# michaelwillett/GPU-ICP-SLAM

Hardware: AMD Instinct MI355X
Metric: particle-scan evals/sec (1081 beams x N particles), full particleFilter step, KD path (higher is better)
Workload: dtype f32; 1 GPU; synthetic 1081-beam scans, 100000 particles/GPU, 100000-point KD map, full SLAM step (disperse+score+weights+ICP/SVD+map update+resample); particles_global=100000, parallelism=particles sharded x1, map replicated, kd_size_end=193011

## Files before the change

gpu-icp-slam_amd/binding.py:

```python
import ctypes as C
import os

import numpy as np

from . import build as _build

NODE_DTYPE = np.dtype(
    [("axis", "<i4"), ("left", "<i4"), ("right", "<i4"), ("parent", "<i4"),
     ("x", "<f4"), ("y", "<f4"), ("z", "<f4"), ("w", "<f4")])
PARTICLE_DTYPE = np.dtype(
    {"names": ["x", "y", "theta", "w", "cluster", "map"],
     "formats": ["<f4", "<f4", "<f4", "<f4", "u1", "<u8"],
     "offsets": [0, 4, 8, 12, 16, 24], "itemsize": 32})

SYMBOLS = [
    "pfslam_default_config", "pfslam_create", "pfslam_destroy", "pfslam_last_error", "pfslam_device_count",
    "pfslam_set_stream", "pfslam_synchronize", "pfslam_step", "pfslam_step_grid", "pfslam_shard_disperse", "pfslam_shard_score", "pfslam_shard_weights", "pfslam_shard_finish", "pfslam_shard_stream", "pfslam_get_pose", "pfslam_get_particles",
    "pfslam_get_map", "pfslam_get_grid", "pfslam_get_trace", "pfslam_get_cells", "pfslam_set_map",
    "pfslam_set_particles", "pfslam_shift_particles", "pfslam_set_scan", "pfslam_set_pose", "pfslam_set_grid", "pfslam_motion_update",
    "pfslam_score_kd", "pfslam_measurement_update", "pfslam_icp", "pfslam_update_map_kd", "pfslam_resample",
    "pfslam_score_grid", "pfslam_update_map_grid", "pfslam_traverse", "pfslam_measurement_local",
    "pfslam_measurement_apply", "pfslam_device_ptr", "pfslam_time_score_kd", "pfslam_set_variant", "pfslam_set_lag",
    "pfslam_kd_create", "pfslam_kd_insert_list", "pfslam_kd_insert_node", "pfslam_kd_balance", "pfslam_set_timing", "pfslam_get_timers", "pfslam_resample_plan", "pfslam_resample_gather", "pfslam_maybe_balance", "pfslam_kd_size", "pfslam_topology_update", "pfslam_find_walls",
    "pfslam_check_loop_closure", "pfslam_get_topology", "pfslam_set_topology", "pfslam_get_closures", "pfslam_score_census", "pfslam_set_census", "pfslam_get_census_log", "pfslam_ubench_gather", "pfslam_plan_stats", "pfslam_cell_stats", "pfslam_kd_parallel_sort", "pfslam_kd_sort_threads", "pfslam_kd_whole_node",
# ... 565 lines not shown

    def traverse(self, xyz):
        xyz = np.ascontiguousarray(xyz, dtype=np.float32).reshape(-1, 3)
        best = np.empty(len(xyz), np.int32)
        _chk(self.L.pfslam_traverse(self._h, _p(xyz), len(xyz), _p(best)), "pfslam_traverse")
        return best

    def debug_math(self, which, x):
        x = np.ascontiguousarray(x, dtype=np.float32).ravel()
        out = np.empty(len(x) * (2 if which in (0, 6, 7) else 1), np.float32)
        _chk(self.L.pfslam_debug_math(self._h, which, _p(x), len(x), _p(out)), "pfslam_debug_math")
        if which == 6:
            return out.view(np.int32).reshape(-1, 2)
        return out.reshape(-1, 2) if which in (0, 7) else out

    @property
    def pose(self):
        out = np.zeros(3, np.float32)
        _chk(self.L.pfslam_get_pose(self._h, _p(out)), "pfslam_get_pose")
        return out

    def particles(self):
        ptr, n = C.c_void_p(), C.c_int()
        _chk(self.L.pfslam_get_particles(self._h, C.byref(ptr), C.byref(n)), "pfslam_get_particles")
        buf = (C.c_char * (32 * n.value)).from_address(ptr.value)
        return np.frombuffer(buf, dtype=PARTICLE_DTYPE).copy()

    def map(self):
        ptr, n = C.c_void_p(), C.c_int()
        _chk(self.L.pfslam_get_map(self._h, C.byref(ptr), C.byref(n)), "pfslam_get_map")
# ... 29 lines not shown
```

gpu-icp-slam_amd/build.py:

```python
import fcntl
import hashlib
import os
import shutil
import subprocess

HERE = os.path.dirname(os.path.abspath(__file__))
CSRC = os.path.join(HERE, "csrc")
OBJ = os.path.join(HERE, "build")
LIB = os.path.join(HERE, "libpfslam_hip.so")
INC = os.path.join("..", "..", "include", "pfslam.h")
UNITS = {
    "pfslam_hip.hip": ["pf_math.h", "kd_device.h", "kd_cells.hip.inc", "pfslam_stages.hip.inc", "pfslam_frame.hip.inc", INC],
    "kd_host.cpp": [INC],
}
FLAGS = ["--offload-arch=gfx950", "-O3", "-std=c++17", "-ffp-contract=off", "-fPIC",
         "-Wall", "-Wno-unused-function", "-Wno-unused-result"] + os.environ.get("PFSLAM_EXTRA_FLAGS", "").split()


def hipcc():
    for c in (os.environ.get("HIPCC"), "/opt/rocm/bin/hipcc", shutil.which("hipcc")):
        if c and os.path.exists(c):
            return c
    raise RuntimeError("hipcc not found: libpfslam_hip.so cannot be built (there is no CPU fallback)")


def _digest(files):
    h = hashlib.sha1(" ".join(FLAGS).encode())
# ... 58 lines not shown
```

gpu-icp-slam_amd/csrc/kd_device.h:

```cpp
#pragma once
#include "pf_math.h"


namespace pf {

struct KdView {
    const uint4 *hot;
    const float *z;
    const int *parent;
    const float *w;
    int planar;
};

struct KdCensus {
    unsigned long long trips;
    unsigned long long lanes;
    unsigned long long tests;
    unsigned long long test_lanes;
    unsigned long long uniform;
    unsigned long long prefix;
    unsigned long long redesc;
    unsigned long long redesc_noop;
};

// ... 30 lines not shown
}
__device__ __forceinline__ int kd_load_i32(kd_rsrc_t r, int idx)
{
    return (int)__builtin_amdgcn_raw_buffer_load_b32(r, idx << 2, 0, 0);
}
__device__ __forceinline__ int kd_load_i32_bytes(kd_rsrc_t r, int byte_offset)
{
    return (int)__builtin_amdgcn_raw_buffer_load_b32(r, byte_offset, 0, 0);
}
__device__ __forceinline__ uint4 kd_load_hot_at(kd_rsrc_t r, int base, int imm)
{
    typedef unsigned u32x4 __attribute__((ext_vector_type(4)));
    const u32x4 v = __builtin_amdgcn_raw_buffer_load_b128(r, base + imm, 0, 0);
    return make_uint4(v.x, v.y, v.z, v.w);
}
#else
struct kd_rsrc_t { const void *base; };
__device__ kd_rsrc_t kd_rsrc(const void *base);
__device__ uint4 kd_load_hot(kd_rsrc_t r, int idx);
__device__ int kd_load_i32(kd_rsrc_t r, int idx);
__device__ int kd_load_i32_bytes(kd_rsrc_t r, int byte_offset);
__device__ uint4 kd_load_hot_at(kd_rsrc_t r, int base, int imm);
#endif

struct KdCensusLocal { unsigned trips, lanes, tests, test_lanes, uniform, prefix, redesc, redesc_noop; };
__device__ __forceinline__ void census_add(unsigned &ev, unsigned &lanes)
{
    const unsigned long long ex = __builtin_amdgcn_read_exec();
    if ((int)(threadIdx.x & 63) == __ffsll((long long)ex) - 1) ev++;
    lanes++;
}
__device__ __forceinline__ void census_flush(const KdCensusLocal &c, KdCensus *out)
{
// ... 110 lines not shown
        if (BOUNDED && head >= bound) head = -1;
        if (CENSUS) {
            in_redesc = true;
            census->redesc++;
        }
    }
    return bestIdx;
}

template <bool PLANAR, bool CENSUS = false>
__device__ __forceinline__ int kd_nearest_ref(const KdView &t, float px, float py, float pz, KdCensusLocal *census = nullptr)
{
    return kd_resume<PLANAR, CENSUS>(t, px, py, pz, INFINITY, 0, 0, census);
}

#define PF_PLAN_CAND 7
struct KdPlanRow {
    int n_cand;
    int resume;
    int path_len;
    float range;
    float4 cand[PF_PLAN_CAND];
};
static_assert(sizeof(KdPlanRow) == 16 + 16 * PF_PLAN_CAND, "plan row layout");

struct KdGroupBox { float xlo, xhi, ylo, yhi, tlo, thi; int count, pad; };

__device__ __forceinline__ float lidar_angle(int n)
{
    const float PI_F = 3.1415926535897932384626422832795028841971f;
// ... 23 lines not shown
```

gpu-icp-slam_amd/csrc/pfslam_frame.hip.inc:

```

#define PF_FRAME_RING 4
enum { PF_FS_BOUND = 0, PF_FS_WALKED = 4, PF_FS_TICKET = 8, PF_FS_ICP = 9, PF_FS_WORDS = 16 };
enum { PF_WC_WALLS = 0, PF_WC_NEW, PF_WC_FLAGS, PF_WC_SIZE, PF_WC_WORDS = 4 };

enum { PF_FL_REDUCED = 0, PF_FL_TREE, PF_FL_ORDER, PF_FL_ICP, PF_FL_SCAN, PF_FL_FTAIL, PF_FL_POSEG , PF_FL_WORDS = 8 };
__device__ __forceinline__ void flag_store(int *word, int ticket) { __hip_atomic_store(word, ticket, __ATOMIC_RELEASE, __HIP_MEMORY_SCOPE_AGENT); }
__device__ __forceinline__ bool flag_wait(const int *word, int ticket, int *err)
{
    const unsigned long long t0 = wall_clock64(), limit = g_gate_ticks;
    while (__hip_atomic_load(word, __ATOMIC_ACQUIRE, __HIP_MEMORY_SCOPE_AGENT) - ticket < 0) {
        __builtin_amdgcn_s_sleep(8);
        if (wall_clock64() - t0 > limit) {
            if (err) __hip_atomic_store(err, ticket, __ATOMIC_RELAXED, __HIP_MEMORY_SCOPE_SYSTEM);
            return false;
        }
    }
    return true;
}
__global__ void k_gate(const int *__restrict__ word, int ticket, int *__restrict__ err)
{
    if (threadIdx.x == 0) flag_wait(word, ticket, err);
}
__global__ void k_gate_signal(int *__restrict__ done_word, int done_ticket, const int *__restrict__ word, int ticket, int *__restrict__ err)
{
// ... 431 lines not shown
#pragma unroll
        for (int q = k >> 1; q > 0; q >>= 1) {
            const uint32_t other = (uint32_t)__shfl_xor((int)key, q, 64);
            const bool asc = (lane & k) == 0, lower = (lane & q) == 0;
            key = (lower == asc) ? min(key, other) : max(key, other);
        }
    runs_g[j] = key;
    keys_s[j] = 0xFFFFFFFFu;
    if (probe && blockIdx.x == 0 && lane == 0) probe[PB_WALLS_KEYS - PB_WALLS] = wall_clock64();
}

template <bool PLANAR>
__global__ __launch_bounds__(64) void k_walls_rank_traverse(const uint32_t *__restrict__ runs_g, int sort_n, const float *__restrict__ pose, int dimx, float resx,
                                                            float resy, float scalex, float scaley, pf::KdView tree, uint32_t *__restrict__ keys_s,
                                                            float2 *__restrict__ xy_s, int *__restrict__ c2_s, int *__restrict__ leaf_s,
                                                            int *__restrict__ new_s, unsigned long long *__restrict__ probe, int split)
{
    pf_stamp(probe);
    extern __shared__ uint32_t s_dyn[];
    uint32_t *runs = s_dyn;
    const int lane = threadIdx.x, n_runs = sort_n >> 6, mine = blockIdx.x / split, per = 64 / split, pos = (blockIdx.x % split) * per + lane;
    for (int i = lane; i < sort_n; i += 64) runs[i] = runs_g[i];
    __syncthreads();
    if (lane >= per) return;
    const int i = mine * 64 + pos;
    const uint32_t key = runs[i];
    if (key == 0xFFFFFFFFu) return;
    int rank = pos;
    bool dup = pos > 0 && runs[i - 1] == key;
    for (int r0 = 0; r0 < n_runs; r0 += 4) {
        int lo[4] = {0, 0, 0, 0};
// ... 9 lines not shown
        for (int step = 32; step >= 1; step >>= 1)
#pragma unroll
            for (int u = 0; u < 4; u++)
                if (on[u]) lo[u] += (runs[(r0 + u) * 64 + lo[u] + step - 1] <= pk[u]) ? step : 0;
#pragma unroll
        for (int u = 0; u < 4; u++)
            if (on[u]) {
                const int cnt = lo[u] + ((lo[u] == 63 && runs[(r0 + u) * 64 + 63] <= pk[u]) ? 1 : 0);
                rank += cnt;
                if (r0 + u < mine && cnt > 0 && runs[(r0 + u) * 64 + cnt - 1] == key) dup = true;
            }
    }
    if (dup) return;
    const float4 p = cell_to_point((int)key, dimx, resx, resy, scalex, scaley, pose[0], pose[1]);
    int leaf;
    const int b = pf::kd_resume<PLANAR, false, true>(tree, p.x, p.y, p.z, INFINITY, 0, 0, nullptr, &leaf);
    const float cellDiag = pf::fsqrt(resx * resx + resy * resy), minDist = cellDiag / 2.0f;
    keys_s[rank] = key;
    xy_s[rank] = make_float2(p.x, p.y);
    c2_s[rank] = b;
    leaf_s[rank] = leaf;
    new_s[rank] = node_dist(tree, b, p) > minDist ? 1 : 0;
}

template <bool PLANAR>
__global__ __launch_bounds__(256) void k_free_traverse(float4 *__restrict__ free_pts, int *__restrict__ free_idx, int free_cap, int wall_cap,
                                                       const int *__restrict__ counts, pf::KdView tree, int zero_tail, float *kw, float resx,
                                                       float resy, const int *__restrict__ bound_ptr, unsigned long long *__restrict__ probe)
{
    pf_stamp(probe);
    const int n_wall = min(counts[0], wall_cap), n_free = min(counts[1], free_cap);
// ... 7 lines not shown
        }
        const int b = pf::kd_resume<PLANAR, false, false, true>(tree, p.x, p.y, p.z, INFINITY, 0, 0, nullptr, nullptr, bound);
        free_idx[i] = b;
        const bool hit = node_dist(tree, b, p) < cellDiag;
        if (zero_tail && i >= n_wall) {
            const unsigned long long m = __ballot(hit);
            if (hit && (int)(threadIdx.x & 63) == __ffsll((long long)m) - 1) map_weight_add(kw, b, PF_FREE_WEIGHT, __popcll(m));
        } else if (hit) map_weight_add(kw, b, PF_FREE_WEIGHT);
    }
}

__global__ __launch_bounds__(1024) void k_wall_weights(const float4 *__restrict__ wall_pts, const int *__restrict__ wall_cell, int wall_cap,
                                                      const int *__restrict__ wall_c2, const int *__restrict__ counts,
                                                      const int *__restrict__ wcounts, pf::KdView tree, float *kw, float resx, float resy,
                                                      const float *__restrict__ pose, HostHeader *__restrict__ hdr, int seq,
                                                      unsigned long long *__restrict__ probe)
{
    pf_stamp(probe);
    const int n_wall = min(counts[0], wall_cap);
    const float cellDiag = pf::fsqrt(resx * resx + resy * resy);
    for (int i = threadIdx.x; i < n_wall; i += 1024) {
        const int b = wall_c2[i];
        if (node_dist(tree, b, wall_pts[i]) < cellDiag) map_weight_add(kw, b, PF_OCCUPIED_WEIGHT);
    }
    if (threadIdx.x != 0 || !hdr) return;
    const int bad = counts[0] != wcounts[PF_WC_WALLS] ? PF_HDR_INTERNAL : 0;
    hdr->n_wall = counts[0];
    hdr->n_free = counts[1];
    hdr->n_new = wcounts[PF_WC_NEW];
    hdr->kd_size = wcounts[PF_WC_SIZE];
    hdr->flags = wcounts[PF_WC_FLAGS] | bad;
    for (int k = 0; k < 4; k++) hdr->pose[k] = pose[k];
    __threadfence_system();
// ... 710 lines not shown
        const int cx = (int)roundf(0.5f * h->dimx + h->cfg.map_res_x / 2), cy = (int)roundf(0.5f * h->dimy + h->cfg.map_res_y / 2);
        const int wait_poseg = c.multi ? 1 : 0;
#define PF_WALLS_ARGS dim3(1), dim3(1024), lds, C, (const float *)h->scan, (const pf::BeamParts *)h->beam_angle, h->nb, sort_n, c.psrc, h->start, h->pose, c.stats_next, \
                      cx, cy, h->dimx, h->dimy, h->cfg.map_res_x, h->cfg.map_res_y, h->cfg.map_scale_x, h->cfg.map_scale_y, c.tv, h->hot, h->parent, h->kz, h->kw,   \
                      h->kd_state, h->kd_cap, sort_n, h->wall_c2, h->wcounts, h->fs + PF_FS_BOUND + ((seq + 1) & 3), (const int *)h->cell_state, h->cell_touched
        if (h->planar == 0) {
            hipLaunchKernelGGL(k_walls<0>, PF_WALLS_ARGS, PB(PB_WALLS), h->wall_xy2, h->wall_leaf2, h->wall_new2, gates ? fl : (int *)nullptr, seq, h->gate_err_dev,
                               (const uint32_t *)nullptr, (const int *)nullptr, wait_poseg, h->trig);
        } else {
            hipLaunchKernelGGL(k_wall_runs, dim3(sort_n / 64), dim3(64), 0, C, (const float *)h->scan, (const pf::BeamParts *)h->beam_angle, h->nb, c.psrc, h->start, h->pose,
                               c.stats_next, cx, cy, h->dimx, h->dimy, h->cfg.map_res_x, h->cfg.map_res_y, h->wall_runs, h->wall_keys_s, PB(PB_WALLS),
                               gates ? fl : (int *)nullptr, seq, h->gate_err_dev, wait_poseg, h->trig);
            const int walls_split = 4;
            hipLaunchKernelGGL(k_walls_rank_traverse<true>, dim3(sort_n / 64 * walls_split), dim3(64), (size_t)sort_n * 4, C, (const uint32_t *)h->wall_runs, sort_n,
                               (const float *)h->pose, h->dimx, h->cfg.map_res_x, h->cfg.map_res_y, h->cfg.map_scale_x, h->cfg.map_scale_y, c.tv, h->wall_keys_s,
                               h->wall_xy2, h->wall_c2s, h->wall_leaf2, h->wall_new2, PB(PB_WALLS_REP), walls_split);
            hipLaunchKernelGGL(k_walls<3>, PF_WALLS_ARGS, PB(PB_WALLS), h->wall_xy2, h->wall_leaf2, h->wall_new2, (int *)nullptr, seq, (int *)nullptr,
                               (const uint32_t *)h->wall_keys_s, (const int *)h->wall_c2s);
        }
#undef PF_WALLS_ARGS
        HIPCHK(hipGetLastError());
        if (!gates) HIPCHK(hipEventRecord(h->ev_tree2, C));
        const int recut = h->cells_passes > 0 && h->cells_passes % PF_CELLS_RECUT_EVERY == 0 ? 1 : 0;
        if (recut) HIPCHK(hipMemsetAsync(h->cell_state + PF_CS_POOL, 0, 4, C));
        hipLaunchKernelGGL(k_cells_update<true>, dim3(PF_CELLS_GRID), dim3(64), 0, C, c.tv, c.geo, h->cell_tab, (const int *)h->cell_list, h->cell_state, h->cell_pool,
                           h->cell_rec, h->cells_gen, (const int *)h->cell_touched, (int)(h->cells_passes & 15), recut, 0,
                           CellPass{nullptr, nullptr, h->fs + PF_FS_WALKED + ((seq - (sync_cells ? 0 : lag)) & 3), nullptr, h->fault}, PB(PB_UPDATE),
                           gates ? fl + PF_FL_TREE : (int *)nullptr, seq);
        HIPCHK(hipGetLastError());
        h->cells_passes++;
    }
// ... 70 lines not shown
        hipLaunchKernelGGL(k_count_cells, dim3(nblk), dim3(256), 0, F, h->free_mask, h->wall_mask, M, h->blk_cnt);
        hipLaunchKernelGGL(k_scatter_cells, dim3(nblk), dim3(256), 0, F, h->free_mask, h->wall_mask, M, h->blk_cnt, h->counts, h->dimx, h->cfg.map_res_x,
                           h->cfg.map_res_y, h->cfg.map_scale_x, h->cfg.map_scale_y, h->pose, h->wall_cell, h->wall_pts, h->max_wall, h->free_cell,
                           h->free_pts, h->max_free, 1, c.psrc);
        h->masks_cleared = true;
        if (h->planar)
            hipLaunchKernelGGL(k_free_traverse<true>, dim3(1024), dim3(256), 0, F, h->free_pts, h->free_c, h->max_free, h->max_wall, (const int *)h->counts, c.tv,
                               h->cfg.free_upload_bug, h->kw, h->cfg.map_res_x, h->cfg.map_res_y, (const int *)(h->fs + PF_FS_BOUND + s4), PB(PB_FREE));
        else
            hipLaunchKernelGGL(k_free_traverse<false>, dim3(1024), dim3(256), 0, F, h->free_pts, h->free_c, h->max_free, h->max_wall, (const int *)h->counts, c.tv,
                               h->cfg.free_upload_bug, h->kw, h->cfg.map_res_x, h->cfg.map_res_y, (const int *)(h->fs + PF_FS_BOUND + s4), PB(PB_FREE));
        HIPCHK(hipGetLastError());
        FV_EDGE_WAIT(F, PF_FL_TREE, h->ev_tree2, 0);
        hipLaunchKernelGGL(k_wall_weights, dim3(1), dim3(1024), 0, F, (const float4 *)h->wall_pts, (const int *)h->wall_cell, h->max_wall, (const int *)h->wall_c2,
                           (const int *)h->counts, (const int *)h->wcounts, c.tv, h->kw, h->cfg.map_res_x, h->cfg.map_res_y, (const float *)h->pose, c.hdr, seq,
                           PB(PB_WALLW));
        HIPCHK(hipGetLastError());
        h->ftail_recorded = !c.ftail_gate;
        if (!c.ftail_gate) HIPCHK(hipEventRecord(h->ev_ftail, F));
    }
    h->pipe_live = true;
    h->plan_valid = false;
    h->cells_valid = true;
    h->mirror_stale = true;
    h->stats_clean = false;
    h->icp_delta_ready = false;
    h->scan_front_done = false;
    pfslam_handle::Frame fr{seq, frame, 0, true, true};
    fr.gtheta = c.multi;
    h->in_flight.push_back(fr);
    while ((int)h->in_flight.size() > (h->topo_in_step == 1 ? 0 : h->lag)) CHK(consume_frame(h));
// ... 14 lines not shown
```

gpu-icp-slam_amd/csrc/pfslam_hip.hip:

```cpp
#include "../../include/pfslam.h"
#include "kd_device.h"
#include "pf_math.h"

#include <hip/hip_runtime.h>

#include <algorithm>
#include <atomic>
#include <deque>
#include <thread>
#include <cmath>
#include <cstdio>
#include <chrono>
#include <cstring>
#include <string>
#include <vector>

#define PF_LIDAR_RANGE 20.0f
#define PF_RANGE_NEVER 28.4f
#define PF_FREE_WEIGHT (-1)
#define PF_OCCUPIED_WEIGHT 4
#define PF_EFFECTIVE_PARTICLES .7
#define PF_CLAMP_VAL 113.0f
#define PF_SVD_EPSILON 0.00001f
#define PF_SUM_TILE 4096
// ... 51 lines not shown
    bool own_stream = false;
    int variant = 0;
    float *pblk = nullptr, *pblk2 = nullptr;
    float *x = nullptr, *y = nullptr, *th = nullptr, *w = nullptr, *wm = nullptr;
    float *x2 = nullptr, *y2 = nullptr, *th2 = nullptr;
    float *gw = nullptr, *gpose = nullptr;
    bool own_global = false;
    long long *gkeys = nullptr, *mkeys = nullptr;
    float *gtheta = nullptr;
    float *scan = nullptr;
    float *scan_base = nullptr;
    int kd_size = 0, kd_cap = 0, planar = 1;
    uint4 *hot = nullptr;
    int *parent = nullptr;
    float *kz = nullptr, *kw = nullptr;
    std::vector<pfslam_node> h_nodes;
    bool integral_w = true;
    float w_absmax = 113.0f;
    float *fit = nullptr, *partial = nullptr;
    size_t partial_elems = 0;
    unsigned *mkey = nullptr;
    int *order2 = nullptr;
    int *cells = nullptr;
    int64_t *stats = nullptr;
    float *pose = nullptr;
    float *start = nullptr;
    float h_pose[3] = {0, 0, 0};
    float *icp_tar = nullptr, *icp_cor = nullptr, *icp_dbg = nullptr;
    uint8_t *free_mask = nullptr, *wall_mask = nullptr;
    int *blk_cnt = nullptr;
// ... 522 lines not shown
    if (i < n) {
        const unsigned c = cell[i];
        order[tile_off[c >> 10] + atomicAdd(&cursor[c], 1)] = i;
    }
}

template <bool PLANAR>
__global__ __launch_bounds__(256) void k_traverse(const float *__restrict__ xyz, int n, pf::KdView tree,
                                                  int *__restrict__ best)
{
    int i = blockIdx.x * 256 + threadIdx.x;
    if (i >= n) return;
    best[i] = pf::kd_nearest_ref<PLANAR>(tree, xyz[3 * i], xyz[3 * i + 1], xyz[3 * i + 2]);
}

__global__ void k_debug_math(int which, const float *__restrict__ in, int n, float *__restrict__ out)
{
    int i = blockIdx.x * blockDim.x + threadIdx.x;
    if (i >= n) return;
    if (which == 0) {
        float s, c;
        pf::sincosf_spec(in[i], s, c);
        out[2 * i] = s;
        out[2 * i + 1] = c;
    } else if (which == 1) {
        out[i] = pf::erfcinvf_spec(in[i]);
    } else if (which == 2) {
        out[i] = pf::asinf_spec(in[i]);
    } else if (which == 3) {
        out[i] = pf::rsqrtf_spec(in[i]);
// ... 119 lines not shown
        CHK(dalloc(&h->gw, (size_t)h->world * S)); CHK(dalloc(&h->gpose, (size_t)h->world * 3 * S));
        h->own_global = true;
        const unsigned long long ticks = PF_GATE_TICKS_SHARDED;
        HIPCHK(hipMemcpyToSymbol(HIP_SYMBOL(g_gate_ticks), &ticks, sizeof(ticks)));
    } else {
        h->gw = h->w;
        h->gpose = h->pblk;
    }
    CHK(dalloc(&h->scan_base, (size_t)h->nb * PF_HDR_SLOTS));
    CHK(dalloc(&h->beam_angle, (size_t)h->nb));
    hipLaunchKernelGGL(k_beam_angles, dim3((h->nb + 255) / 256), dim3(256), 0, h->stream, h->beam_angle, h->nb);
    HIPCHK(hipGetLastError());
    h->scan = h->scan_base;
    CHK(dalloc(&h->hot, (size_t)h->kd_cap)); CHK(dalloc(&h->parent, (size_t)h->kd_cap));
    CHK(dalloc(&h->kz, (size_t)h->kd_cap)); CHK(dalloc(&h->kw, (size_t)h->kd_cap));
    CHK(dalloc(&h->fit, n)); CHK(dalloc(&h->fit_i, n));
    CHK(dalloc(&h->mkey, n)); CHK(dalloc(&h->order2, n));
    CHK(dalloc(&h->cells, (size_t)2 * PF_CELLS_MAX + PF_CELLS_MAX / 1024));
    HIPCHK(hipMemsetAsync(h->cells, 0, ((size_t)2 * PF_CELLS_MAX + PF_CELLS_MAX / 1024) * sizeof(int), h->stream));
    CHK(dalloc(&h->stats, 8)); CHK(dalloc(&h->pose, 4)); CHK(dalloc(&h->start, 4));
    CHK(dalloc(&h->icp_tar, (size_t)h->nb * 4)); CHK(dalloc(&h->icp_cor, (size_t)h->nb * 4)); CHK(dalloc(&h->icp_dbg, 64));
    CHK(dalloc(&h->free_mask, 2 * M));
    h->wall_mask = h->free_mask + M;
    h->max_wall = h->nb;
    h->max_free = (int)std::min<size_t>(M, (size_t)h->nb * (size_t)std::max(h->dimx, h->dimy));
    CHK(dalloc(&h->blk_cnt, 2 * ((M + 4095) / 4096) + 8));
    CHK(dalloc(&h->wall_cell, (size_t)h->max_wall)); CHK(dalloc(&h->free_cell, (size_t)h->max_free));
    CHK(dalloc(&h->wall_pts, (size_t)h->max_wall)); CHK(dalloc(&h->free_pts, (size_t)h->max_free));
    CHK(dalloc(&h->wall_c, (size_t)h->max_wall)); CHK(dalloc(&h->free_c, (size_t)h->max_free));
    CHK(dalloc(&h->counts, 8));
// ... 65 lines not shown
        const std::string msg = g_err;
        pfslam_destroy(h);
        g_err = msg;
        return rc;
    }
    *out = h;
    return 0;
}

extern "C" int pfslam_destroy(pfslam_handle *h)
{
    if (!h) return 0;
    (void)hipSetDevice(h->cfg.device);
    (void)settle(h);
    if (h->stream) (void)hipStreamSynchronize(h->stream);
    void *bufs[] = {h->pblk, h->pblk2, h->w, h->wm, h->gkeys, h->mkeys, h->gtheta, h->scan_base, h->hot, h->parent, h->kz, h->kw,
                    h->fit, h->fit_i, h->partial, h->mkey, h->order2, h->cells, h->stats, h->pose, h->start, h->icp_tar, h->icp_cor, h->icp_dbg,
                    h->free_mask, h->blk_cnt, h->wall_cell, h->free_cell, h->wall_pts, h->free_pts,
                    h->wall_c, h->free_c, h->counts, h->tile_r, h->tile_r2, h->sums, h->cdf,
                    h->chunk_max, h->tile_tot, h->tile_off, h->tile_pmax, h->src, h->est_part, h->grid, h->d_count, h->wall_leaf, h->kd_state, h->d_sigma};
    for (void *b : bufs)
        if (b) (void)hipFree(b);
    if (h->own_global) {
        (void)hipFree(h->gw); (void)hipFree(h->gpose);
    }
    if (h->pin_tree) (void)hipHostFree(h->pin_tree);
    if (h->h_hdr) (void)hipHostFree(h->h_hdr);
    if (h->h_scan) (void)hipHostFree(h->h_scan);
    if (h->ev0) (void)hipEventDestroy(h->ev0);
    if (h->ev1) (void)hipEventDestroy(h->ev1);
    if (h->aux) { (void)hipStreamSynchronize(h->aux); (void)hipStreamDestroy(h->aux); }
// ... 140 lines not shown
    const int per = (n + nt - 1) / nt;
    for (int t = 0; t < nt; t++) th.emplace_back([=] { fn(std::min(n, t * per), std::min(n, (t + 1) * per), t); });
    for (auto &t : th) t.join();
}

static int upload_tree(pfslam_handle *h, const pfslam_node *nodes, int n, std::vector<pfslam_node> *own = nullptr)
{
    if (n > h->kd_cap) return fail("map larger than kd_capacity");
    if (n == 0) {
        h->h_nodes.clear();
        h->kd_size = 0;
        h->mirror_n = 0;
        h->mirror_stale = false;
        h->cells_wipe_pending = true;
        HIPCHK(hipMemsetAsync(h->kd_state, 0, 16, h->stream));
        HIPCHK(hipStreamSynchronize(h->stream));
        return 0;
    }
    std::vector<uint4> hot_v;
    std::vector<int> par_v;
    std::vector<float> z_v, w_v;
    if (!h->pin_tree) {
        void *p = nullptr;
        if (hipHostMalloc(&p, (size_t)h->kd_cap * 28, hipHostMallocDefault) == hipSuccess) h->pin_tree = p;
        else (void)hipGetLastError();
    }
    uint4 *hot;
    int *par;
    float *z, *w;
    if (h->pin_tree) {
// ... 52 lines not shown
            if (planar && nd.axis == 2) memcpy(&z[i], &nd.left, 4);
        }
    });
    HIPCHK(hipMemcpyAsync(h->hot, hot, (size_t)n * 16, hipMemcpyHostToDevice, h->stream));
    HIPCHK(hipMemcpyAsync(h->parent, par, (size_t)n * 4, hipMemcpyHostToDevice, h->stream));
    HIPCHK(hipMemcpyAsync(h->kz, z, (size_t)n * 4, hipMemcpyHostToDevice, h->stream));
    HIPCHK(hipMemcpyAsync(h->kw, w, (size_t)n * 4, hipMemcpyHostToDevice, h->stream));
    float wabs;
    {
        const int wb = wmax_bits.load();
        memcpy(&wabs, &wb, 4);
        wabs = std::max(wabs, PF_CLAMP_VAL);
    }
    const int state[4] = {n, planar, integral ? (int)std::min(wabs, 1e9f) : 0, lattice ? 1 : 0};
    HIPCHK(hipMemcpyAsync(h->kd_state, state, 16, hipMemcpyHostToDevice, h->stream));
    if (own && own->data() == nodes && (int)own->size() == n) h->h_nodes.swap(*own);
    else h->h_nodes.assign(nodes, nodes + n);
    HIPCHK(hipStreamSynchronize(h->stream));
    h->kd_size = n;
    h->mirror_n = n;
    h->mirror_stale = false;
    h->planar = planar;
    h->integral_w = integral;
    h->w_absmax = wabs;
    h->lattice_ok = lattice;
    h->cells_wipe_pending = true;
    h->pipe_live = false;
    h->cells_suspended = false;
    h->cells_full_frame = -1;
    return 0;
// ... 923 lines not shown
    CHK(settle(h));
    const int per = which == 0 || which == 6 || which == 7 ? 2 : 1;
    float *d_in = nullptr, *d_out = nullptr;
    CHK(dalloc(&d_in, (size_t)n));
    CHK(dalloc(&d_out, (size_t)n * per));
    HIPCHK(hipMemcpyAsync(d_in, in_host, (size_t)n * 4, hipMemcpyHostToDevice, h->stream));
    hipLaunchKernelGGL(k_debug_math, dim3((n + 255) / 256), dim3(256), 0, h->stream, which, d_in, n, d_out);
    HIPCHK(hipGetLastError());
    HIPCHK(hipMemcpyAsync(out_host, d_out, (size_t)n * per * 4, hipMemcpyDeviceToHost, h->stream));
    HIPCHK(hipStreamSynchronize(h->stream));
    HIPCHK(hipFree(d_in));
    HIPCHK(hipFree(d_out));
    return 0;
}

extern "C" int pfslam_device_ptr(pfslam_handle *h, int which, void **ptr, size_t *bytes)
{
    if (!h || !ptr || !bytes) return fail("pfslam_device_ptr: bad argument");
    const size_t n = h->n;
    switch (which) {
    case 0: *ptr = h->stats; *bytes = 64; break;
    case 1: *ptr = h->fit; *bytes = n * 4; break;
    case 2: *ptr = h->x; *bytes = n * 4; break;
    case 3: *ptr = h->y; *bytes = n * 4; break;
    case 4: *ptr = h->th; *bytes = n * 4; break;
    case 5: *ptr = h->w; *bytes = (size_t)h->stride * 4; break;
    case 6: *ptr = h->tile_r; *bytes = ((n + PF_SUM_TILE - 1) / PF_SUM_TILE) * 4; break;
    case 7: *ptr = h->scan; *bytes = (size_t)h->nb * 4; break;
    case 8: *ptr = h->start; *bytes = 16; break;
    case 9: *ptr = h->pose; *bytes = 16; break;
// ... 26 lines not shown
```

gpu-icp-slam_amd/csrc/pfslam_stages.hip.inc:

```

__device__ __forceinline__ long long wave_max_i64(long long v)
{
    for (int off = 32; off >= 1; off >>= 1) {
        long long o = __shfl_xor(v, off, 64);
        v = o > v ? o : v;
    }
    return v;
}
__device__ __forceinline__ float wave_max_f32(float v)
{
    for (int off = 32; off >= 1; off >>= 1) v = fmaxf(v, __shfl_xor(v, off, 64));
    return v;
}
template <typename F>
__device__ __forceinline__ float wave_sum_canonical(int n, F elem)
{
    const int lane = threadIdx.x & 63;
    float acc = 0.0f;
    for (int i = lane; i < n; i += 64) acc = acc + elem(i);
    for (int off = 32; off >= 1; off >>= 1) acc = acc + __shfl_xor(acc, off, 64);
    return acc;
}

__device__ __forceinline__ int f32_to_ordered(float f)
// ... 2548 lines not shown
    return rc;
}
extern "C" int pfslam_shard_balance_adopt(pfslam_handle *h)
{
    if (!h) return fail("null handle");
    HIPCHK(hipSetDevice(h->cfg.device));
    CHK(settle(h));
    int st[4] = {0, 0, 0, 0};
    HIPCHK(hipMemcpyAsync(st, h->kd_state, 16, hipMemcpyDeviceToHost, h->stream));
    HIPCHK(hipStreamSynchronize(h->stream));
    if (st[0] != h->kd_size) return fail("pfslam_shard_balance_adopt: the broadcast map has " + std::to_string(st[0]) + " nodes, this rank's " + std::to_string(h->kd_size));
    h->planar = st[1];
    h->integral_w = st[2] != 0;
    h->w_absmax = st[2] != 0 ? (float)st[2] : 113.0f;
    h->lattice_ok = st[3] != 0;
    h->mirror_n = 0;
    h->mirror_stale = true;
    h->cells_wipe_pending = true;
    return 0;
}

extern "C" int pfslam_maybe_balance(pfslam_handle *h, int frame)
{
    if (!h) return fail("null handle");
    HIPCHK(hipSetDevice(h->cfg.device));
    CHK(settle(h));
    return balance_if_due(h, frame);
}
extern "C" int pfslam_kd_size(pfslam_handle *h)
{
// ... 231 lines not shown
```

gpu-icp-slam_amd/csrc/pfslam_testhooks.h:

```cpp
#ifndef PFSLAM_TESTHOOKS_H
#define PFSLAM_TESTHOOKS_H
#include "../../include/pfslam.h"
#ifdef __cplusplus
extern "C" {
#endif
int pfslam_debug_math(pfslam_handle *h, int which, const float *in_host, int n, float *out_host);
#ifdef __cplusplus
}
#endif
#endif
```

Before: 173.5 million particle-scan evals/s.

## Prefetch grandchild nodes via hint table in wall-rank KD traversal

Adds a per-node hint table holding grandchild indices. The table is rebuilt when the map is set or adopted and patched incrementally after inserts in the wall-weights kernel. The wall-rank traversal kernel now uses a paired walk that loads the next node and both candidate grandchildren in parallel, which shortens the chain of dependent loads in the KD descent. In exchange it issues more memory traffic per step, adds hint maintenance work, and depends on the hints staying current after tree updates.

```diff
diff --git a/gpu-icp-slam_amd/binding.py b/gpu-icp-slam_amd/binding.py
--- a/gpu-icp-slam_amd/binding.py
+++ b/gpu-icp-slam_amd/binding.py
@@ -603,6 +603,21 @@
             return out.view(np.int32).reshape(-1, 2)
         return out.reshape(-1, 2) if which in (0, 7) else out
 
+    def debug_walk_paired(self, xyz, hint_mode=0):
+        xyz = np.ascontiguousarray(xyz, dtype=np.float32).reshape(-1, 3)
+        out = [np.empty(len(xyz), np.int32) for _ in range(4)]
+        f = self.L.pfslam_debug_walk_paired
+        f.argtypes = [C.c_void_p, C.c_void_p, C.c_int, C.c_int] + [C.c_void_p] * 4
+        _chk(f(self._h, _p(xyz), len(xyz), hint_mode, *[_p(o) for o in out]), "pfslam_debug_walk_paired")
+        return tuple(out)
+
+    def debug_hints(self):
+        out = np.zeros(3, np.int64)
+        f = self.L.pfslam_debug_hints
+        f.argtypes = [C.c_void_p, C.c_void_p]
+        _chk(f(self._h, _p(out)), "pfslam_debug_hints")
+        return int(out[0]), int(out[1]), int(out[2])
+
     @property
     def pose(self):
         out = np.zeros(3, np.float32)
diff --git a/gpu-icp-slam_amd/build.py b/gpu-icp-slam_amd/build.py
--- a/gpu-icp-slam_amd/build.py
+++ b/gpu-icp-slam_amd/build.py
@@ -10,7 +10,7 @@
 LIB = os.path.join(HERE, "libpfslam_hip.so")
 INC = os.path.join("..", "..", "include", "pfslam.h")
 UNITS = {
-    "pfslam_hip.hip": ["pf_math.h", "kd_device.h", "kd_cells.hip.inc", "pfslam_stages.hip.inc", "pfslam_frame.hip.inc", INC],
+    "pfslam_hip.hip": ["pf_math.h", "kd_device.h", "kd_hint.h", "kd_cells.hip.inc", "pfslam_stages.hip.inc", "pfslam_frame.hip.inc", INC],
     "kd_host.cpp": [INC],
 }
 FLAGS = ["--offload-arch=gfx950", "-O3", "-std=c++17", "-ffp-contract=off", "-fPIC",
diff --git a/gpu-icp-slam_amd/csrc/kd_device.h b/gpu-icp-slam_amd/csrc/kd_device.h
--- a/gpu-icp-slam_amd/csrc/kd_device.h
+++ b/gpu-icp-slam_amd/csrc/kd_device.h
@@ -1,5 +1,6 @@
 #pragma once
 #include "pf_math.h"
+#include "kd_hint.h"
 
 
 namespace pf {
@@ -68,9 +69,21 @@
     const u32x4 v = __builtin_amdgcn_raw_buffer_load_b128(r, base + imm, 0, 0);
     return make_uint4(v.x, v.y, v.z, v.w);
 }
+__device__ __forceinline__ kd_rsrc_t kd_rsrc_n(const void *base, unsigned bytes)
+{
+    return __builtin_amdgcn_make_buffer_rsrc(const_cast<void *>(base),  0, (int)bytes, 0x00020000);
+}
+__device__ __forceinline__ int4 kd_load_hint(kd_rsrc_t r, int idx)
+{
+    typedef unsigned u32x4 __attribute__((ext_vector_type(4)));
+    const u32x4 v = __builtin_amdgcn_raw_buffer_load_b128(r, idx << 4, 0, 0);
+    return make_int4((int)v.x, (int)v.y, (int)v.z, (int)v.w);
+}
 #else
 struct kd_rsrc_t { const void *base; };
 __device__ kd_rsrc_t kd_rsrc(const void *base);
+__device__ kd_rsrc_t kd_rsrc_n(const void *base, unsigned bytes);
+__device__ int4 kd_load_hint(kd_rsrc_t r, int idx);
 __device__ uint4 kd_load_hot(kd_rsrc_t r, int idx);
 __device__ int kd_load_i32(kd_rsrc_t r, int idx);
 __device__ int kd_load_i32_bytes(kd_rsrc_t r, int byte_offset);
@@ -211,6 +224,128 @@
     return kd_resume<PLANAR, CENSUS>(t, px, py, pz, INFINITY, 0, 0, census);
 }
 
+struct KdStep { uint4 rec; int zw; int4 hint; int idx; };
+
+template <bool PLANAR>
+__device__ __forceinline__ int kd_walk_paired(const KdView &t, const int4 *hint, int cap, float px, float py, float pz, int *leaf_slot)
+{
+    const kd_rsrc_t hot_rsrc = kd_rsrc_n(t.hot, (unsigned)cap * 16u), z_rsrc = kd_rsrc_n(t.z, (unsigned)cap * 4u),
+                    hint_rsrc = kd_rsrc_n(hint, (unsigned)cap * 16u);
+    auto fetch = [&](int i) {
+        KdStep s;
+        s.rec = kd_load_hot(hot_rsrc, i);
+        s.zw = kd_load_i32(z_rsrc, i);
+        s.hint = kd_load_hint(hint_rsrc, i);
+        s.idx = i;
+        return s;
+    };
+    float sBest = INFINITY;
+    int bestIdx = 0, prevBest = -1, leaf = -1;
+    bool leaf_open = true;
+    bool went_left = false;
+    KdStep prev = {make_uint4(0u, 0u, 0u, 0u), 0, make_int4(-1, -1, -1, -1), -1};
+    KdStep par = prev;
+    auto visit = [&](const KdStep &n) -> int {
+        const uint4 nd = n.rec;
+        const int head = n.idx;
+        typedef float f32x2 __attribute__((ext_vector_type(2)));
+        const f32x2 nxy = {__uint_as_float(nd.x), __uint_as_float(nd.y)};
+        const f32x2 pxy = {px, py};
+        const f32x2 d = nxy - pxy;
+        const f32x2 dd = d * d;
+        float s = dd.x + dd.y;
+        float dz = 0.0f;
+        int zleft = 0;
+        if (!PLANAR) {
+            const float zraw = __int_as_float(n.zw);
+            const float nz = t.planar ? 0.0f : zraw;
+            zleft = n.zw;
+            dz = nz - pz;
+            s = s + dz * dz;
+        }
+        const float sGuard = sBest * PF_GUARD_K;
+        bool take = s < sGuard;
+        const bool inBand = (s < sBest) != take;
+        if (__builtin_amdgcn_ballot_w64(inBand) != 0ull) {
+            float sb = sBest;
+            asm volatile("" : "+v"(sb));
+            take = take | (inBand && fsqrt(s) < fsqrt(sb));
+        }
+        sBest = take ? s : sBest;
+        bestIdx = take ? head : bestIdx;
+        if (take) par = prev;
+        const uint32_t axis = nd.z >> 30;
+        float da = axis == 0 ? d.x : d.y;
+        if (!PLANAR) da = axis == 2 ? dz : da;
+        const bool lt = da > 0.0f;
+        int left = hot_left(nd.z);
+        if (!PLANAR) left = (t.planar && axis == 2) ? zleft : left;
+        if (leaf_open) leaf = head * 2 + ((lt && !(PLANAR && axis == 2)) ? 0 : 1);
+        prev = n;
+        went_left = lt;
+        return lt ? left : (int)nd.w;
+    };
+    const KdStep root = fetch(0);
+    int c = visit(root);
+    int pL = went_left ? root.hint.x : root.hint.z, pR = went_left ? root.hint.y : root.hint.w;
+    for (;;) {
+        while (c >= 0) {
+            const KdStep a = fetch(c), l = fetch(pL < 0 ? 0 : pL), r = fetch(pR < 0 ? 0 : pR);
+            const int g = visit(a);
+            if (g < 0) break;
+            KdStep b;
+            if (g == pL) b = l;
+            else if (g == pR) b = r;
+            else b = fetch(g);
+            c = visit(b);
+            pL = went_left ? b.hint.x : b.hint.z;
+            pR = went_left ? b.hint.y : b.hint.w;
+        }
+        if (leaf_open) {
+            leaf_open = false;
+            *leaf_slot = leaf;
+        }
+        if (bestIdx == prevBest) break;
+        prevBest = bestIdx;
+        const float bestDist = fsqrt(sBest);
+        if (par.idx < 0) break;
+        const uint4 nd = par.rec;
+        const float nx = __uint_as_float(nd.x), ny = __uint_as_float(nd.y);
+        const uint32_t axis = nd.z >> 30;
+        float pa = axis == 0 ? px : py, na = axis == 0 ? nx : ny;
+        float hd;
+        bool lt;
+        int left = hot_left(nd.z);
+        bool true_left = false;
+        if (PLANAR) {
+            hd = axis < 2 ? fabsf(pa - na) : 0.0f;
+            lt = (pa < na) & (axis < 2);
+            if (axis == 2) {
+                left = par.zw;
+                true_left = true;
+            }
+        } else {
+            if (axis == 2) {
+                const float zraw = __int_as_float(par.zw);
+                pa = pz;
+                na = t.planar ? 0.0f : zraw;
+                if (t.planar) {
+                    left = par.zw;
+                    true_left = true;
+                }
+            }
+            hd = fabsf(pa - na);
+            lt = pa < na;
+        }
+        if (!(hd < bestDist)) break;
+        c = lt ? (int)nd.w : left;
+        pL = lt ? par.hint.z : true_left ? -1 : par.hint.x;
+        pR = lt ? par.hint.w : true_left ? -1 : par.hint.y;
+        prev = par;
+    }
+    return bestIdx;
+}
+
 #define PF_PLAN_CAND 7
 struct KdPlanRow {
     int n_cand;
diff --git a/gpu-icp-slam_amd/csrc/kd_hint.h b/gpu-icp-slam_amd/csrc/kd_hint.h
--- /dev/null
+++ b/gpu-icp-slam_amd/csrc/kd_hint.h
@@ -0,0 +1,28 @@
+#pragma once
+#include <stdint.h>
+
+#if defined(__HIPCC__)
+#define KD_HINT_HD __host__ __device__ __forceinline__
+#else
+#define KD_HINT_HD inline
+#endif
+
+struct KdHint { int ll, lr, rl, rr; };
+
+KD_HINT_HD int kd_hint_left(uint32_t la) { return ((int)(la << 2)) >> 2; }
+
+template <class Hot>
+KD_HINT_HD KdHint kd_hint_from_links(const Hot *hot, int n)
+{
+    const int L = kd_hint_left(hot[n].z), R = (int)hot[n].w;
+    KdHint h = {-1, -1, -1, -1};
+    if (L >= 0) {
+        h.ll = kd_hint_left(hot[L].z);
+        h.lr = (int)hot[L].w;
+    }
+    if (R >= 0) {
+        h.rl = kd_hint_left(hot[R].z);
+        h.rr = (int)hot[R].w;
+    }
+    return h;
+}
diff --git a/gpu-icp-slam_amd/csrc/pfslam_frame.hip.inc b/gpu-icp-slam_amd/csrc/pfslam_frame.hip.inc
--- a/gpu-icp-slam_amd/csrc/pfslam_frame.hip.inc
+++ b/gpu-icp-slam_amd/csrc/pfslam_frame.hip.inc
@@ -469,7 +469,8 @@
 __global__ __launch_bounds__(64) void k_walls_rank_traverse(const uint32_t *__restrict__ runs_g, int sort_n, const float *__restrict__ pose, int dimx, float resx,
                                                             float resy, float scalex, float scaley, pf::KdView tree, uint32_t *__restrict__ keys_s,
                                                             float2 *__restrict__ xy_s, int *__restrict__ c2_s, int *__restrict__ leaf_s,
-                                                            int *__restrict__ new_s, unsigned long long *__restrict__ probe, int split)
+                                                            int *__restrict__ new_s, unsigned long long *__restrict__ probe, int split,
+                                                            const int4 *__restrict__ hint, int kd_cap)
 {
     pf_stamp(probe);
     extern __shared__ uint32_t s_dyn[];
@@ -509,7 +510,7 @@
     if (dup) return;
     const float4 p = cell_to_point((int)key, dimx, resx, resy, scalex, scaley, pose[0], pose[1]);
     int leaf;
-    const int b = pf::kd_resume<PLANAR, false, true>(tree, p.x, p.y, p.z, INFINITY, 0, 0, nullptr, &leaf);
+    const int b = pf::kd_walk_paired<PLANAR>(tree, hint, kd_cap, p.x, p.y, p.z, &leaf);
     const float cellDiag = pf::fsqrt(resx * resx + resy * resy), minDist = cellDiag / 2.0f;
     keys_s[rank] = key;
     xy_s[rank] = make_float2(p.x, p.y);
@@ -547,9 +548,21 @@
                                                       const int *__restrict__ wall_c2, const int *__restrict__ counts,
                                                       const int *__restrict__ wcounts, pf::KdView tree, float *kw, float resx, float resy,
                                                       const float *__restrict__ pose, HostHeader *__restrict__ hdr, int seq,
-                                                      unsigned long long *__restrict__ probe)
+                                                      unsigned long long *__restrict__ probe, int4 *__restrict__ hint, const int *__restrict__ old_size)
 {
     pf_stamp(probe);
+    if (hint) {
+        const int v0 = *old_size, v1 = wcounts[PF_WC_SIZE];
+        for (int v = v0 + (int)threadIdx.x; v < v1; v += 1024) {
+            const KdHint hv = kd_hint_from_links(tree.hot, v);
+            hint[v] = make_int4(hv.ll, hv.lr, hv.rl, hv.rr);
+            const int p = tree.parent[v], q = p >= 0 ? tree.parent[p] : -1;
+            if (q >= 0) {
+                const KdHint hq = kd_hint_from_links(tree.hot, q);
+                hint[q] = make_int4(hq.ll, hq.lr, hq.rl, hq.rr);
+            }
+        }
+    }
     const int n_wall = min(counts[0], wall_cap);
     const float cellDiag = pf::fsqrt(resx * resx + resy * resy);
     for (int i = threadIdx.x; i < n_wall; i += 1024) {
@@ -1290,7 +1303,7 @@
             const int walls_split = 4;
             hipLaunchKernelGGL(k_walls_rank_traverse<true>, dim3(sort_n / 64 * walls_split), dim3(64), (size_t)sort_n * 4, C, (const uint32_t *)h->wall_runs, sort_n,
                                (const float *)h->pose, h->dimx, h->cfg.map_res_x, h->cfg.map_res_y, h->cfg.map_scale_x, h->cfg.map_scale_y, c.tv, h->wall_keys_s,
-                               h->wall_xy2, h->wall_c2s, h->wall_leaf2, h->wall_new2, PB(PB_WALLS_REP), walls_split);
+                               h->wall_xy2, h->wall_c2s, h->wall_leaf2, h->wall_new2, PB(PB_WALLS_REP), walls_split, (const int4 *)h->kd_hint, h->kd_cap);
             hipLaunchKernelGGL(k_walls<3>, PF_WALLS_ARGS, PB(PB_WALLS), h->wall_xy2, h->wall_leaf2, h->wall_new2, (int *)nullptr, seq, (int *)nullptr,
                                (const uint32_t *)h->wall_keys_s, (const int *)h->wall_c2s);
         }
@@ -1391,7 +1404,7 @@
         FV_EDGE_WAIT(F, PF_FL_TREE, h->ev_tree2, 0);
         hipLaunchKernelGGL(k_wall_weights, dim3(1), dim3(1024), 0, F, (const float4 *)h->wall_pts, (const int *)h->wall_cell, h->max_wall, (const int *)h->wall_c2,
                            (const int *)h->counts, (const int *)h->wcounts, c.tv, h->kw, h->cfg.map_res_x, h->cfg.map_res_y, (const float *)h->pose, c.hdr, seq,
-                           PB(PB_WALLW));
+                           PB(PB_WALLW), h->kd_hint, (const int *)(h->fs + PF_FS_BOUND + s4));
         HIPCHK(hipGetLastError());
         h->ftail_recorded = !c.ftail_gate;
         if (!c.ftail_gate) HIPCHK(hipEventRecord(h->ev_ftail, F));
diff --git a/gpu-icp-slam_amd/csrc/pfslam_hip.hip b/gpu-icp-slam_amd/csrc/pfslam_hip.hip
--- a/gpu-icp-slam_amd/csrc/pfslam_hip.hip
+++ b/gpu-icp-slam_amd/csrc/pfslam_hip.hip
@@ -89,6 +89,8 @@
     uint4 *hot = nullptr;
     int *parent = nullptr;
     float *kz = nullptr, *kw = nullptr;
+    int kd_size_hi = 0;
+    int4 *kd_hint = nullptr;
     std::vector<pfslam_node> h_nodes;
     bool integral_w = true;
     float w_absmax = 113.0f;
@@ -641,6 +643,64 @@
     best[i] = pf::kd_nearest_ref<PLANAR>(tree, xyz[3 * i], xyz[3 * i + 1], xyz[3 * i + 2]);
 }
 
+__global__ __launch_bounds__(256) void k_kd_hints(const uint4 *__restrict__ hot, int4 *__restrict__ hint, int n, int n_clear)
+{
+    const int i = blockIdx.x * 256 + threadIdx.x;
+    if (i >= n_clear) return;
+    KdHint v = {-1, -1, -1, -1};
+    if (i < n) v = kd_hint_from_links(hot, i);
+    hint[i] = make_int4(v.ll, v.lr, v.rl, v.rr);
+}
+static int build_hints(pfslam_handle *h, int n, int n_clear, hipStream_t s)
+{
+    n_clear = std::min(std::max(n, n_clear), h->kd_cap);
+    if (n_clear <= 0) return 0;
+    hipLaunchKernelGGL(k_kd_hints, dim3((n_clear + 255) / 256), dim3(256), 0, s, (const uint4 *)h->hot, h->kd_hint, n, n_clear);
+    HIPCHK(hipGetLastError());
+    return 0;
+}
+template <bool PLANAR>
+__global__ __launch_bounds__(256) void k_debug_walk_paired(const float *__restrict__ xyz, int n, pf::KdView tree, const int4 *__restrict__ hint, int cap,
+                                                           int *__restrict__ best_plain, int *__restrict__ leaf_plain, int *__restrict__ best_paired,
+                                                           int *__restrict__ leaf_paired)
+{
+    const int i = blockIdx.x * 256 + threadIdx.x;
+    if (i >= n) return;
+    const float px = xyz[3 * i], py = xyz[3 * i + 1], pz = xyz[3 * i + 2];
+    int la = -1, lb = -1;
+    best_plain[i] = pf::kd_resume<PLANAR, false, true>(tree, px, py, pz, INFINITY, 0, 0, nullptr, &la);
+    best_paired[i] = pf::kd_walk_paired<PLANAR>(tree, hint, cap, px, py, pz, &lb);
+    leaf_plain[i] = la;
+    leaf_paired[i] = lb;
+}
+__global__ __launch_bounds__(256) void k_hints_scramble(int4 *__restrict__ hint, int n, unsigned seed)
+{
+    const int i = blockIdx.x * 256 + threadIdx.x;
+    if (i >= n) return;
+    int v[4];
+    for (int k = 0; k < 4; k++) {
+        unsigned x = (unsigned)(4 * i + k) * 2654435761u + seed;
+        x ^= x >> 15; x *= 2246822519u; x ^= x >> 13;
+        v[k] = (int)(x % (unsigned)n);
+    }
+    hint[i] = make_int4(v[0], v[1], v[2], v[3]);
+}
+__global__ __launch_bounds__(256) void k_hints_check(const uint4 *__restrict__ hot, const int4 *__restrict__ hint, int n, unsigned long long *__restrict__ out)
+{
+    const int i = blockIdx.x * 256 + threadIdx.x;
+    if (i >= n) return;
+    const KdHint v = kd_hint_from_links(hot, i);
+    const int4 g = hint[i];
+    const int want[4] = {v.ll, v.lr, v.rl, v.rr}, got[4] = {g.x, g.y, g.z, g.w};
+    int stale = 0, missing = 0;
+    for (int k = 0; k < 4; k++) {
+        stale += got[k] != want[k] ? 1 : 0;
+        missing += (got[k] == -1 && want[k] != -1) ? 1 : 0;
+    }
+    if (stale) atomicAdd(&out[0], (unsigned long long)stale);
+    if (missing) atomicAdd(&out[1], (unsigned long long)missing);
+}
+
 __global__ void k_debug_math(int which, const float *__restrict__ in, int n, float *__restrict__ out)
 {
     int i = blockIdx.x * blockDim.x + threadIdx.x;
@@ -790,6 +850,8 @@
     h->scan = h->scan_base;
     CHK(dalloc(&h->hot, (size_t)h->kd_cap)); CHK(dalloc(&h->parent, (size_t)h->kd_cap));
     CHK(dalloc(&h->kz, (size_t)h->kd_cap)); CHK(dalloc(&h->kw, (size_t)h->kd_cap));
+    CHK(dalloc(&h->kd_hint, (size_t)h->kd_cap));
+    HIPCHK(hipMemsetAsync(h->kd_hint, 0xFF, (size_t)h->kd_cap * sizeof(int4), h->stream));
     CHK(dalloc(&h->fit, n)); CHK(dalloc(&h->fit_i, n));
     CHK(dalloc(&h->mkey, n)); CHK(dalloc(&h->order2, n));
     CHK(dalloc(&h->cells, (size_t)2 * PF_CELLS_MAX + PF_CELLS_MAX / 1024));
@@ -885,7 +947,7 @@
     (void)hipSetDevice(h->cfg.device);
     (void)settle(h);
     if (h->stream) (void)hipStreamSynchronize(h->stream);
-    void *bufs[] = {h->pblk, h->pblk2, h->w, h->wm, h->gkeys, h->mkeys, h->gtheta, h->scan_base, h->hot, h->parent, h->kz, h->kw,
+    void *bufs[] = {h->pblk, h->pblk2, h->w, h->wm, h->gkeys, h->mkeys, h->gtheta, h->scan_base, h->hot, h->parent, h->kz, h->kw, h->kd_hint,
                     h->fit, h->fit_i, h->partial, h->mkey, h->order2, h->cells, h->stats, h->pose, h->start, h->icp_tar, h->icp_cor, h->icp_dbg,
                     h->free_mask, h->blk_cnt, h->wall_cell, h->free_cell, h->wall_pts, h->free_pts,
                     h->wall_c, h->free_c, h->counts, h->tile_r, h->tile_r2, h->sums, h->cdf,
@@ -1056,6 +1118,8 @@
         h->mirror_stale = false;
         h->cells_wipe_pending = true;
         HIPCHK(hipMemsetAsync(h->kd_state, 0, 16, h->stream));
+        CHK(build_hints(h, 0, h->kd_size_hi, h->stream));
+        h->kd_size_hi = 0;
         HIPCHK(hipStreamSynchronize(h->stream));
         return 0;
     }
@@ -1138,6 +1202,8 @@
     }
     const int state[4] = {n, planar, integral ? (int)std::min(wabs, 1e9f) : 0, lattice ? 1 : 0};
     HIPCHK(hipMemcpyAsync(h->kd_state, state, 16, hipMemcpyHostToDevice, h->stream));
+    CHK(build_hints(h, n, std::max(h->kd_size, h->kd_size_hi), h->stream));
+    h->kd_size_hi = n;
     if (own && own->data() == nodes && (int)own->size() == n) h->h_nodes.swap(*own);
     else h->h_nodes.assign(nodes, nodes + n);
     HIPCHK(hipStreamSynchronize(h->stream));
@@ -2091,6 +2157,68 @@
     return 0;
 }
 
+extern "C" int pfslam_debug_walk_paired(pfslam_handle *h, const float *xyz_host, int n, int hint_mode, int32_t *best_plain, int32_t *leaf_plain,
+                                        int32_t *best_paired, int32_t *leaf_paired)
+{
+    if (!h || !xyz_host || n <= 0 || hint_mode < 0 || hint_mode > 2 || !best_plain || !leaf_plain || !best_paired || !leaf_paired)
+        return fail("pfslam_debug_walk_paired: bad argument");
+    HIPCHK(hipSetDevice(h->cfg.device));
+    CHK(settle(h));
+    const int size = h->kd_size;
+    if (size <= 0) return fail("pfslam_debug_walk_paired: no map");
+    float *d_xyz = nullptr;
+    int *d_out = nullptr;
+    int4 *d_hint = nullptr;
+    CHK(dalloc(&d_xyz, (size_t)n * 3));
+    CHK(dalloc(&d_out, (size_t)n * 4));
+    const int4 *hint = h->kd_hint;
+    if (hint_mode != 0) {
+        CHK(dalloc(&d_hint, (size_t)size));
+        if (hint_mode == 1) HIPCHK(hipMemsetAsync(d_hint, 0xFF, (size_t)size * sizeof(int4), h->stream));
+        else hipLaunchKernelGGL(k_hints_scramble, dim3((size + 255) / 256), dim3(256), 0, h->stream, d_hint, size, 0x9E3779B9u);
+        hint = d_hint;
+    }
+    HIPCHK(hipMemcpyAsync(d_xyz, xyz_host, (size_t)n * 12, hipMemcpyHostToDevice, h->stream));
+    if (h->planar)
+        hipLaunchKernelGGL(k_debug_walk_paired<true>, dim3((n + 255) / 256), dim3(256), 0, h->stream, d_xyz, n, kd_view(h), hint, size, d_out, d_out + n,
+                           d_out + 2 * n, d_out + 3 * n);
+    else
+        hipLaunchKernelGGL(k_debug_walk_paired<false>, dim3((n + 255) / 256), dim3(256), 0, h->stream, d_xyz, n, kd_view(h), hint, size, d_out, d_out + n,
+                           d_out + 2 * n, d_out + 3 * n);
+    HIPCHK(hipGetLastError());
+    HIPCHK(hipMemcpyAsync(best_plain, d_out, (size_t)n * 4, hipMemcpyDeviceToHost, h->stream));
+    HIPCHK(hipMemcpyAsync(leaf_plain, d_out + n, (size_t)n * 4, hipMemcpyDeviceToHost, h->stream));
+    HIPCHK(hipMemcpyAsync(best_paired, d_out + 2 * n, (size_t)n * 4, hipMemcpyDeviceToHost, h->stream));
+    HIPCHK(hipMemcpyAsync(leaf_paired, d_out + 3 * n, (size_t)n * 4, hipMemcpyDeviceToHost, h->stream));
+    HIPCHK(hipStreamSynchronize(h->stream));
+    HIPCHK(hipFree(d_xyz));
+    HIPCHK(hipFree(d_out));
+    if (d_hint) HIPCHK(hipFree(d_hint));
+    return 0;
+}
+
+extern "C" int pfslam_debug_hints(pfslam_handle *h, long long out[3])
+{
+    if (!h || !out) return fail("pfslam_debug_hints: bad argument");
+    HIPCHK(hipSetDevice(h->cfg.device));
+    CHK(settle(h));
+    const int size = h->kd_size;
+    out[0] = size;
+    out[1] = out[2] = 0;
+    if (size <= 0) return 0;
+    unsigned long long *d_cnt = nullptr, cnt[2] = {0, 0};
+    CHK(dalloc(&d_cnt, 2));
+    HIPCHK(hipMemsetAsync(d_cnt, 0, 16, h->stream));
+    hipLaunchKernelGGL(k_hints_check, dim3((size + 255) / 256), dim3(256), 0, h->stream, (const uint4 *)h->hot, (const int4 *)h->kd_hint, size, d_cnt);
+    HIPCHK(hipGetLastError());
+    HIPCHK(hipMemcpyAsync(cnt, d_cnt, 16, hipMemcpyDeviceToHost, h->stream));
+    HIPCHK(hipStreamSynchronize(h->stream));
+    HIPCHK(hipFree(d_cnt));
+    out[1] = (long long)cnt[0];
+    out[2] = (long long)cnt[1];
+    return 0;
+}
+
 extern "C" int pfslam_device_ptr(pfslam_handle *h, int which, void **ptr, size_t *bytes)
 {
     if (!h || !ptr || !bytes) return fail("pfslam_device_ptr: bad argument");
diff --git a/gpu-icp-slam_amd/csrc/pfslam_stages.hip.inc b/gpu-icp-slam_amd/csrc/pfslam_stages.hip.inc
--- a/gpu-icp-slam_amd/csrc/pfslam_stages.hip.inc
+++ b/gpu-icp-slam_amd/csrc/pfslam_stages.hip.inc
@@ -2586,6 +2586,9 @@
     h->integral_w = st[2] != 0;
     h->w_absmax = st[2] != 0 ? (float)st[2] : 113.0f;
     h->lattice_ok = st[3] != 0;
+    CHK(build_hints(h, st[0], h->kd_size_hi, h->stream));
+    HIPCHK(hipStreamSynchronize(h->stream));
+    h->kd_size_hi = st[0];
     h->mirror_n = 0;
     h->mirror_stale = true;
     h->cells_wipe_pending = true;
diff --git a/gpu-icp-slam_amd/csrc/pfslam_testhooks.h b/gpu-icp-slam_amd/csrc/pfslam_testhooks.h
--- a/gpu-icp-slam_amd/csrc/pfslam_testhooks.h
+++ b/gpu-icp-slam_amd/csrc/pfslam_testhooks.h
@@ -5,6 +5,9 @@
 extern "C" {
 #endif
 int pfslam_debug_math(pfslam_handle *h, int which, const float *in_host, int n, float *out_host);
+int pfslam_debug_walk_paired(pfslam_handle *h, const float *xyz_host, int n, int hint_mode, int32_t *best_plain, int32_t *leaf_plain,
+                             int32_t *best_paired, int32_t *leaf_paired);
+int pfslam_debug_hints(pfslam_handle *h, long long out[3]);
 #ifdef __cplusplus
 }
 #endif
```

Measured after the change: 173.1 million particle-scan evals/s, median of 2. About the same (-0.2%).
